# CornellHPC/HySortK

Measured on AMD Instinct MI355X. Metric: k-mers counted/sec at K=31, higher is better.
Workload: dtype u64

## Files before the change

hysortk_amd/csrc/hsk_device.h:

```cpp
#pragma once
#include <hip/hip_runtime.h>
#include <stdint.h>
#include "hsk_passplan.h"

namespace hsk {

typedef uint64_t u64;
typedef uint32_t u32;
typedef uint16_t u16;
typedef uint8_t u8;

constexpr int WAVE = 64;

__host__ __device__ __forceinline__ u64 rotl64(u64 x, int r) { return (x << r) | (x >> (64 - r)); }
__host__ __device__ __forceinline__ u64 fmix64(u64 k)
{
    k ^= k >> 33; k *= 0xff51afd7ed558ccdULL; k ^= k >> 33; k *= 0xc4ceb9fe1a85ec53ULL; k ^= k >> 33;
    return k;
}
__host__ __device__ __forceinline__ u64 murmur64_8(u64 key)
{
    u64 k1 = key * 0x87c37b91114253d5ULL;
    k1 = rotl64(k1, 31);
    k1 *= 0x4cf5ad432745937fULL;
    u64 h1 = 313ULL ^ k1, h2 = 313ULL;
    h1 ^= 8; h2 ^= 8;
    h1 += h2; h2 += h1;
    h1 = fmix64(h1); h2 = fmix64(h2);
    return h1 + h2;
}

template <int NW>
__host__ __device__ __forceinline__ u64 murmur64_words(const u64 (&w)[NW])
{
    if (NW == 1) return murmur64_8(w[0]);
    const u64 c1 = 0x87c37b91114253d5ULL, c2 = 0x4cf5ad432745937fULL;
    u64 h1 = 313ULL, h2 = 313ULL;
    u64 k1 = w[0], k2 = w[NW > 1 ? 1 : 0];
    k1 *= c1; k1 = rotl64(k1, 31); k1 *= c2; h1 ^= k1;
    h1 = rotl64(h1, 27); h1 += h2; h1 = h1 * 5 + 0x52dce729ULL;
    k2 *= c2; k2 = rotl64(k2, 33); k2 *= c1; h2 ^= k2;
    h2 = rotl64(h2, 31); h2 += h1; h2 = h2 * 5 + 0x38495ab5ULL;
    if (NW == 3) { u64 t1 = w[NW > 2 ? 2 : 0]; t1 *= c1; t1 = rotl64(t1, 31); t1 *= c2; h1 ^= t1; }
    h1 ^= (u64)(8 * NW); h2 ^= (u64)(8 * NW);
    h1 += h2; h2 += h1;
    h1 = fmix64(h1); h2 = fmix64(h2);
    return h1 + h2;
}

__host__ __device__ __forceinline__ u64 rev2(u64 x)
{
#if defined(__HIP_DEVICE_COMPILE__)
    x = __brevll(x);
#else
    x = ((x >> 1) & 0x5555555555555555ULL) | ((x & 0x5555555555555555ULL) << 1);
    x = ((x >> 2) & 0x3333333333333333ULL) | ((x & 0x3333333333333333ULL) << 2);
    x = ((x >> 4) & 0x0f0f0f0f0f0f0f0fULL) | ((x & 0x0f0f0f0f0f0f0f0fULL) << 4);
    x = __builtin_bswap64(x);
#endif
    return ((x >> 1) & 0x5555555555555555ULL) | ((x & 0x5555555555555555ULL) << 1);
}

__host__ __device__ __forceinline__ u64 twin1(u64 fw, int len)
{
    u64 t = ~rev2(fw);
    return t << (64 - 2 * len);
}

template <int NW> struct Mer { u64 w[NW]; };

template <int NW>
__host__ __device__ __forceinline__ Mer<NW> twin(const Mer<NW> &m, int k)
{
    Mer<NW> t;
#pragma unroll
    for (int l = 0; l < NW; ++l) t.w[NW - 1 - l] = ~rev2(m.w[l]);
    const int sh = (NW * 64 - 2 * k);
    if (sh) {
#pragma unroll
        for (int i = 0; i < NW; ++i) {
            u64 nxt = (i + 1 < NW) ? t.w[i + 1] : 0;
            t.w[i] = (t.w[i] << sh) | (nxt >> (64 - sh));
        }
    }
    return t;
}

template <int NW>
__host__ __device__ __forceinline__ bool mer_less(const Mer<NW> &a, const Mer<NW> &b)
{
#pragma unroll
    for (int i = 0; i < NW; ++i) {
        if (a.w[i] < b.w[i]) return true;
        if (a.w[i] > b.w[i]) return false;
    }
    return false;
}

template <int NW>
__host__ __device__ __forceinline__ Mer<NW> canonical(const Mer<NW> &m, int k)
{
    Mer<NW> t = twin<NW>(m, k);
    return mer_less<NW>(t, m) ? t : m;
}

__device__ __forceinline__ u64 bits64_be32(const u32 *words, u32 bit)
{
    u32 i = bit >> 5, s = bit & 31;
    u64 hi = ((u64)words[i] << 32) | words[i + 1];
    u64 lo = (u64)words[i + 2] << 32;
    return s ? ((hi << s) | (lo >> (64 - s))) : hi;
}

__device__ __forceinline__ u64 bits64_bytes(const u64 *p8, u64 bit)
{
    u64 i = bit >> 6; u32 s = (u32)(bit & 63);
    u64 hi = __builtin_bswap64(p8[i]);
    if (!s) return hi;
    u64 lo = __builtin_bswap64(p8[i + 1]);
    return (hi << s) | (lo >> (64 - s));
}
__device__ __forceinline__ u64 bits64_bytes_clamped(const u64 *p8, u64 bit, u64 nwords)
{
    u64 i = bit >> 6; u32 s = (u32)(bit & 63);
    u64 hi = i < nwords ? __builtin_bswap64(p8[i]) : 0;
    if (!s) return hi;
    u64 lo = (i + 1 < nwords) ? __builtin_bswap64(p8[i + 1]) : 0;
    return (hi << s) | (lo >> (64 - s));
}

struct FastMod { u32 d; u32 c16, c32, c48; u32 inv; };
inline FastMod make_fastmod(u32 d)
{
    FastMod f; f.d = d;
    f.c16 = d > 1 ? (u32)((1ULL << 16) % d) : 0; f.c32 = d > 1 ? (u32)((1ULL << 32) % d) : 0; f.c48 = d > 1 ? (u32)((1ULL << 48) % d) : 0;
    f.inv = d > 1 ? (u32)((1ULL << 32) / d) : 0;
    return f;
}
__host__ __device__ __forceinline__ u32 fastmod64(u64 x, const FastMod &f)
{
    if (f.d <= 1) return 0;
    const u32 a = (u32)(x >> 48), b = (u32)(x >> 32) & 0xFFFFu, c = (u32)(x >> 16) & 0xFFFFu, e = (u32)x & 0xFFFFu;
    const u32 t = a * f.c48 + b * f.c32 + c * f.c16 + e;
#if defined(__HIP_DEVICE_COMPILE__)
    const u32 q = __umulhi(t, f.inv);
#else
    const u32 q = (u32)(((u64)t * f.inv) >> 32);
#endif
    u32 r = t - q * f.d;
    if (r >= f.d) r -= f.d;
    if (r >= f.d) r -= f.d;
    return r;
}

__device__ __forceinline__ int lane_id() { return (int)__builtin_amdgcn_mbcnt_hi(~0u, __builtin_amdgcn_mbcnt_lo(~0u, 0)); }

__device__ __forceinline__ u32 wave_incl_scan_dpp(u32 v)
{
    v += (u32)__builtin_amdgcn_update_dpp(0, (int)v, 0x111, 0xF, 0xF, false);
    v += (u32)__builtin_amdgcn_update_dpp(0, (int)v, 0x112, 0xF, 0xF, false);
    v += (u32)__builtin_amdgcn_update_dpp(0, (int)v, 0x114, 0xF, 0xF, false);
    v += (u32)__builtin_amdgcn_update_dpp(0, (int)v, 0x118, 0xF, 0xF, false);
    v += (u32)__builtin_amdgcn_update_dpp(0, (int)v, 0x142, 0xA, 0xF, false);
    v += (u32)__builtin_amdgcn_update_dpp(0, (int)v, 0x143, 0xC, 0xF, false);
    return v;
}

template <typename T>
__device__ __forceinline__ T wave_incl_scan(T v)
{
    if constexpr (sizeof(T) == 4 && (T)(-1) > (T)0) return (T)wave_incl_scan_dpp((u32)v);
    const int lane = lane_id();
#pragma unroll
    for (int o = 1; o < WAVE; o <<= 1) {
        T n = __shfl_up(v, o, WAVE);
        if (lane >= o) v += n;
    }
    return v;
}

template <typename T>
__device__ __forceinline__ T block_excl_scan_256(T v, T *scratch, T *total)
{
    const int lane = lane_id(), w = threadIdx.x >> 6;
    T inc = wave_incl_scan(v);
    if (lane == WAVE - 1) scratch[w] = inc;
    __syncthreads();
    T base = 0, tot = 0;
#pragma unroll
    for (int i = 0; i < 4; ++i) { T s = scratch[i]; if (i < w) base += s; tot += s; }
    __syncthreads();
    if (total) *total = tot;
    return base + inc - v;
}

__device__ __forceinline__ void lds_barrier() { asm volatile("s_waitcnt lgkmcnt(0)\n\ts_barrier" ::: "memory"); }

template <typename T>
__device__ __forceinline__ T block_excl_scan_256_lds(T v, T *scratch, T *total)
{
    const int lane = lane_id(), w = threadIdx.x >> 6;
    T inc = wave_incl_scan(v);
    if (lane == WAVE - 1) scratch[w] = inc;
    lds_barrier();
    T base = 0, tot = 0;
#pragma unroll
    for (int i = 0; i < 4; ++i) { T s = scratch[i]; if (i < w) base += s; tot += s; }
    lds_barrier();
    if (total) *total = tot;
    return base + inc - v;
}


template <int NW> __device__ __forceinline__ u64 pick_word(const u64 *k, int word)
{
    if (NW == 1) return k[0];
    if (NW == 2) return word == 0 ? k[0] : k[1];
    return word == 0 ? k[0] : (word == 1 ? k[1] : k[NW - 1]);
}

__host__ __device__ __forceinline__ u64 splitmix64(u64 x)
{
    x += 0x9e3779b97f4a7c15ULL;
    x = (x ^ (x >> 30)) * 0xbf58476d1ce4e5b9ULL;
    x = (x ^ (x >> 27)) * 0x94d049bb133111ebULL;
    return x ^ (x >> 31);
}

}
```

hysortk_amd/csrc/hsk_parse.h:

```cpp
#pragma once
#include "hsk_device.h"
#include "hsk_parseplan.h"

namespace hsk {

constexpr int PARSE_THREADS = 256;
constexpr int PARSE_PPT = 8;
static_assert(PARSE_TILE == PARSE_THREADS * PARSE_PPT, "a tile is one pass of the workgroup: 2048 positions = 512 bytes");
constexpr int SUPERMER_CUT = 128;
constexpr int MAX_K = 95;
constexpr int HSK_MAX_TASKS = 1024;
constexpr int PARSE_HMAX = PARSE_TILE + 96;
constexpr int PARSE_RWIN = 64;
static_assert(PARSE_RWIN + PARSE_WORDS <= PARSE_THREADS, "scan_kernel prefetches the next tile with one lane per read-index entry and per word");

struct BinTable { u32 *cursor; u32 *map; u32 vmax; u32 cap_chunks; u32 *ctl; u32 *chunk_bin; ulonglong2 *items; u32 *subs; u32 *err; };

struct ParseArgs {
    const u8 *packed;
    u64 packed_bytes;
    const u64 *roff;
    const u32 *rlen;
    u64 nreads;
    int k, m;
    u32 ntasks;
    FastMod fm;
    u64 ntiles;
    u32 tiles_per_block;
    u32 nslabs, slab;
    u64 slab_tiles;
    u32 place_one;
    int64_t rid_base;
    u64 *blk_cnt;
    const u64 *blk_base;
    u8 *sm_len;
    u64 *sm_gpos;
    int32_t *dump_dest;
    u16 *dest_cache;
    u32 *tile_rec;
    u32 *tile_nrec;
    u32 rec_cap;
    u32 place_group;
    u32 *overflow;
    u32 *tile_r0;
    u32 *tile_sub;
    u32 *sm_sub;
    u32 item_maxk;
    const struct BinTable *bins;
    unsigned short *sm_sub16;
    u32 vt_shift;
    u64 *sm_item;
    const u8 *task_skip;
    u8 *sm_bytes;
    u32 *sm_boff;
    const u64 *task_base3;
    u32 *packed_copy;
    u32 drop_mask;
    unsigned long long *dropped;
};

enum ParseMode { PARSE_COUNT = 0, PARSE_EMIT = 1, PARSE_DUMP = 2 };

__device__ __forceinline__ u64 find_read(const u64 *roff, u64 lo, u64 hi, u64 b)
{
    while (lo < hi) {
        u64 mid = lo + (hi - lo + 1) / 2;
        if (roff[mid] <= b) lo = mid; else hi = mid - 1;
    }
    return lo;
}

__device__ __forceinline__ void supermer_runs(const u16 *s_dest, u64 *s_bnd, u32 (&runs)[PARSE_PPT])
{
    const int tid = threadIdx.x, lane = tid & 63, wave = tid >> 6;
    bool start[PARSE_PPT];
#pragma unroll
    for (int j = 0; j < PARSE_PPT; ++j) {
        const u32 p = j * PARSE_THREADS + tid;
        const u16 d = s_dest[p];
        const u16 dp = p ? s_dest[p - 1] : (u16)0xFFFF;
        const bool bnd = (d == 0xFFFF) || ((p & (SUPERMER_CUT - 1)) == 0) || (d != dp);
        start[j] = bnd && d != 0xFFFF;
        const u64 m = __ballot(bnd);
        if (lane == 0) s_bnd[j * 4 + wave] = m;
    }
    __syncthreads();
#pragma unroll
    for (int j = 0; j < PARSE_PPT; ++j) {
        runs[j] = 0;
        if (!start[j]) continue;
        const u32 p = j * PARSE_THREADS + tid;
        const u32 lim = (p | (SUPERMER_CUT - 1)) + 1;
        const u32 w = p >> 6;
        u64 m = ((p & 63) == 63) ? 0ULL : (s_bnd[w] & (~0ULL << ((p & 63) + 1)));
        u32 nb = lim;
        if (m) nb = w * 64 + (u32)__builtin_ctzll(m);
        else if ((w & 1) == 0) { const u64 m2 = s_bnd[w + 1]; if (m2) nb = (w + 1) * 64 + (u32)__builtin_ctzll(m2); }
        runs[j] = nb - p;
    }
}

template <int MW>
__device__ __forceinline__ u64 wide_mmer_hash(const u32 *s_words, u32 p, int M)
{
    Mer<MW> fw;
#pragma unroll
    for (int x = 0; x < MW; ++x) fw.w[x] = bits64_be32(s_words, 2u * p + 64u * (u32)x);
    fw.w[MW - 1] &= ~0ULL << (64 * MW - 2 * M);
    const Mer<MW> c = canonical<MW>(fw, M);
    return murmur64_words<MW>(c.w);
}

__device__ __forceinline__ u32 homopolymer_positions(const u32 *s_words, int tid, int K, u32 drop_mask)
{
    const u64 d0 = bits64_be32(s_words, 16u * (u32)tid), d1 = bits64_be32(s_words, 16u * (u32)tid + 64u);
    u32 dm = 0;
#pragma unroll
    for (int i = 0; i < PARSE_PPT; ++i) {
        const u64 hi = i ? ((d0 << (2 * i)) | (d1 >> (64 - 2 * i))) : d0, lo = d1 << (2 * i);
        const u32 b = (u32)(hi >> 62);
        const u64 pat = ((b & 1u) ? 0x5555555555555555ULL : 0ULL) | ((b & 2u) ? 0xAAAAAAAAAAAAAAAAULL : 0ULL);
        const bool same = K <= 32 ? ((hi ^ pat) >> (64 - 2 * K)) == 0 : (hi == pat && ((lo ^ pat) >> (128 - 2 * K)) == 0);
        if (same && ((drop_mask >> ((b == 1u || b == 2u) ? 1 : 0)) & 1u)) dm |= 1u << i;
    }
    return dm;
}

template <int MODE, bool EXT, bool DROP = false>
__global__ __launch_bounds__(PARSE_THREADS, 4) void parse_kernel(ParseArgs a)
{
    __shared__ u32 s_words[PARSE_WORDS];
    __shared__ u64 s_hash[PARSE_HMAX];
    __shared__ __attribute__((aligned(16))) u16 s_dest[PARSE_TILE + 8];
    __shared__ u64 s_rng[4];
    __shared__ u64 s_roff[PARSE_RWIN];
    __shared__ u32 s_rlen[PARSE_RWIN];
    __shared__ u64 s_bnd[PARSE_TILE / 64];
    __shared__ u32 s_scan[12];
    extern __shared__ __attribute__((aligned(16))) u64 s_cur[];

    u32 ndrop = 0;
    const int tid = threadIdx.x;
    const int K = a.k, M = a.m, W = K - M + 1;
    const u64 total_pos = a.packed_bytes * 4;

    if (MODE == PARSE_COUNT) {
        for (u32 i = tid; i < 2 * a.ntasks; i += PARSE_THREADS) s_cur[i] = 0;
    } else if (MODE == PARSE_EMIT) {
        for (u32 t = tid; t < a.ntasks; t += PARSE_THREADS) s_cur[t] = a.blk_base[((u64)blockIdx.x * a.ntasks + t) * 2];
    }
    __syncthreads();

    const u64 tile0 = (u64)blockIdx.x * a.tiles_per_block;
    if (tid == 0) s_rng[1] = (tile0 < a.ntiles) ? find_read(a.roff, 0, a.nreads - 1, (tile0 * PARSE_TILE) >> 2) : 0;
    __syncthreads();
    const u64 RINF = ~0ULL >> 2;
    for (u32 ti = 0; ti < a.tiles_per_block; ++ti) {
        const u64 tile = tile0 + ti;
        if (tile >= a.ntiles) break;
        const u64 gbase = tile * PARSE_TILE;
        const bool cached_emit = (MODE == PARSE_EMIT) && a.dest_cache != nullptr;
        const u64 bbase = gbase >> 2;

        if (!cached_emit) {
            const u32 *src = reinterpret_cast<const u32 *>(a.packed + bbase);
            const u64 left = a.packed_bytes - bbase;
            for (int i = tid; i < PARSE_WORDS; i += PARSE_THREADS) {
                u32 wv = 0;
                if ((u64)i * 4 + 4 <= left) wv = __builtin_bswap32(src[i]);
                else if ((u64)i * 4 < left) {
                    for (u64 b = (u64)i * 4; b < left; ++b) wv |= (u32)a.packed[bbase + b] << (24 - 8 * (b & 3));
                }
                s_words[i] = wv;
            }
        }
        if (!cached_emit && tid < PARSE_RWIN) {
            const u64 rb = s_rng[1];
            u64 blast = bbase + PARSE_TILE / 4 - 1;
            if (blast >= a.packed_bytes) blast = a.packed_bytes - 1;
            const u64 idx = rb + tid;
            const u64 off = (idx <= a.nreads) ? a.roff[idx] : RINF;
            s_roff[tid] = off;
            s_rlen[tid] = (idx < a.nreads) ? a.rlen[idx] : 0;
            const u32 c0 = (u32)__popcll(__ballot(idx < a.nreads && off <= bbase));
            const u32 c1 = (u32)__popcll(__ballot(idx < a.nreads && off <= blast));
            if (tid == 0) {
                u64 r0 = rb + c0 - 1, r1 = rb + c1 - 1;
                const bool fast = c1 < PARSE_RWIN;
                if (!fast) {
                    r0 = find_read(a.roff, rb, a.nreads - 1, bbase);
                    r1 = find_read(a.roff, r0, a.nreads - 1, blast);
                }
                s_rng[0] = r0; s_rng[1] = r1; s_rng[2] = rb; s_rng[3] = fast ? 1 : 0;
            }
        }
        __syncthreads();

        const int p0 = tid * PARSE_PPT;
        const bool cached = cached_emit;
        const u64 mmask = ~0ULL << (64 - 2 * (M < 32 ? M : 31));
        if (!cached) {
            if (M < 32) {
                for (int p = tid; p < PARSE_TILE + W - 1; p += PARSE_THREADS) {
                    u64 fw = bits64_be32(s_words, 2u * (u32)p) & mmask;
                    u64 tw = twin1(fw, M);
                    s_hash[p] = murmur64_8(tw < fw ? tw : fw);
                }
            } else if (M < 64) {
                for (int p = tid; p < PARSE_TILE + W - 1; p += PARSE_THREADS) s_hash[p] = wide_mmer_hash<2>(s_words, (u32)p, M);
            } else {
                for (int p = tid; p < PARSE_TILE + W - 1; p += PARSE_THREADS) s_hash[p] = wide_mmer_hash<3>(s_words, (u32)p, M);
            }
        }
        __syncthreads();

        u64 mn[PARSE_PPT];
        if (cached) {
#pragma unroll
            for (int i = 0; i < PARSE_PPT; ++i) mn[i] = 0;
        } else if (W >= PARSE_PPT) {
            u64 c = ~0ULL;
            for (int j = PARSE_PPT - 1; j <= W - 1; ++j) { u64 v = s_hash[p0 + j]; c = v < c ? v : c; }
            u64 suf = ~0ULL;
            mn[PARSE_PPT - 1] = c;
#pragma unroll
            for (int i = PARSE_PPT - 2; i >= 0; --i) { u64 v = s_hash[p0 + i]; suf = v < suf ? v : suf; mn[i] = suf < c ? suf : c; }
            u64 run = ~0ULL;
#pragma unroll
            for (int i = 1; i < PARSE_PPT; ++i) { u64 v = s_hash[p0 + W + i - 1]; run = v < run ? v : run; mn[i] = run < mn[i] ? run : mn[i]; }
        } else {
#pragma unroll
            for (int i = 0; i < PARSE_PPT; ++i) {
                u64 c = ~0ULL;
                for (int j = 0; j < W; ++j) { u64 v = s_hash[p0 + i + j]; c = v < c ? v : c; }
                mn[i] = c;
            }
        }
        if (!cached) {
            const u64 g0 = gbase + p0;
            const u64 rlo = s_rng[0], rhi = s_rng[1], rb = s_rng[2];
            const bool fast = s_rng[3] != 0;
            u64 r, rstart, rend, nxt;
            if (fast) {
                u32 lo = (u32)(rlo - rb), hi = (u32)(rhi - rb);
                const u64 b0 = g0 >> 2;
                while (lo < hi) { u32 mid = (lo + hi + 1) >> 1; if (s_roff[mid] <= b0) lo = mid; else hi = mid - 1; }
                r = rb + lo; rstart = s_roff[lo] * 4; rend = rstart + s_rlen[lo];
                nxt = (r + 1 < a.nreads) ? s_roff[lo + 1] * 4 : ~0ULL;
            } else {
                r = find_read(a.roff, rlo, rhi, g0 >> 2);
                rstart = a.roff[r] * 4; rend = rstart + a.rlen[r];
                nxt = (r + 1 < a.nreads) ? a.roff[r + 1] * 4 : ~0ULL;
            }
            const int HUGE = 1 << 30;
            auto rel = [&](u64 x) -> int { return x >= gbase + (u64)HUGE ? HUGE : (x < gbase ? ((gbase - x) >= (u64)HUGE ? -HUGE : -(int)(gbase - x)) : (int)(x - gbase)); };
            int rend_r = rel(rend), nxt_r = rel(nxt);
            const int total_r = rel(total_pos);
            u32 dmk = 0;
            if constexpr (DROP) dmk = homopolymer_positions(s_words, tid, K, a.drop_mask);
#pragma unroll
            for (int i = 0; i < PARSE_PPT; ++i) {
                const int g = p0 + i;
                while (g >= nxt_r) {
                    ++r; rstart = nxt;
                    if (fast) { const u32 j = (u32)(r - rb); rend = rstart + s_rlen[j]; nxt = (r + 1 < a.nreads) ? s_roff[j + 1] * 4 : ~0ULL; }
                    else { rend = rstart + a.rlen[r]; nxt = (r + 1 < a.nreads) ? a.roff[r + 1] * 4 : ~0ULL; }
                    rend_r = rel(rend); nxt_r = rel(nxt);
                }
                bool valid = (g < total_r) && (g + K <= rend_r);
                if (DROP && valid && ((dmk >> i) & 1u)) { valid = false; if (MODE == PARSE_COUNT) ++ndrop; }
                const u32 d = fastmod64(mn[i], a.fm);
                s_dest[p0 + i] = valid ? (u16)d : (u16)0xFFFF;
            }
        }
        if (cached) {
            const uint4 v = *reinterpret_cast<const uint4 *>(a.dest_cache + gbase + p0);
            *reinterpret_cast<uint4 *>(&s_dest[p0]) = v;
        } else if (MODE == PARSE_COUNT && a.dest_cache != nullptr) {
            *reinterpret_cast<uint4 *>(a.dest_cache + gbase + p0) = *reinterpret_cast<const uint4 *>(&s_dest[p0]);
        }
        __syncthreads();

        if (MODE == PARSE_DUMP) {
#pragma unroll
            for (int i = 0; i < PARSE_PPT; ++i) {
                u64 g = gbase + p0 + i;
                if (g < total_pos) { u16 d = s_dest[p0 + i]; a.dump_dest[g] = d == 0xFFFF ? -1 : (int32_t)d; }
            }
        } else if (MODE == PARSE_COUNT) {
            u32 runs[PARSE_PPT];
            supermer_runs(s_dest, s_bnd, runs);
#pragma unroll
            for (int j = 0; j < PARSE_PPT; ++j) {
                if (!runs[j]) continue;
                const u32 d = s_dest[j * PARSE_THREADS + tid];
                const u32 nk = runs[j];
                const u32 nb = (nk + K - 1 + 3) >> 2;
                atomicAdd((unsigned long long *)&s_cur[2 * d + 0], (1ULL << 40) | (unsigned long long)nk);
                atomicAdd((unsigned long long *)&s_cur[2 * d + 1], (unsigned long long)nb);
            }
        } else {
            u32 *s_srt = reinterpret_cast<u32 *>(s_hash);
            u32 *s_tcnt = reinterpret_cast<u32 *>(s_cur + a.ntasks);
            u32 *s_tpre = s_tcnt + a.ntasks;
            for (u32 t = tid; t < a.ntasks; t += PARSE_THREADS) s_tcnt[t] = 0;
            __syncthreads();
            u32 rec[PARSE_PPT], rnk[PARSE_PPT];
            {
                u32 runs[PARSE_PPT];
                supermer_runs(s_dest, s_bnd, runs);
#pragma unroll
                for (int j = 0; j < PARSE_PPT; ++j) {
                    rec[j] = 0xFFFFFFFFu;
                    if (!runs[j]) continue;
                    const u32 p = j * PARSE_THREADS + tid;
                    const u32 d = s_dest[p];
                    rec[j] = p | ((runs[j] - 1) << 11) | (d << 18);
                    rnk[j] = atomicAdd(&s_tcnt[d], 1u);
                }
            }
            __syncthreads();
            {
                u32 c4[4], sum = 0;
#pragma unroll
                for (int j = 0; j < 4; ++j) { const u32 t = tid * 4 + j; c4[j] = t < a.ntasks ? s_tcnt[t] : 0; sum += c4[j]; }
                u32 tot;
                u32 e = block_excl_scan_256<u32>(sum, s_scan, &tot);
#pragma unroll
                for (int j = 0; j < 4; ++j) { const u32 t = tid * 4 + j; if (t < a.ntasks) s_tpre[t] = e; e += c4[j]; }
                if (tid == 0) s_scan[8] = tot;
            }
            __syncthreads();
#pragma unroll
            for (int i = 0; i < PARSE_PPT; ++i)
                if (rec[i] != 0xFFFFFFFFu) s_srt[s_tpre[rec[i] >> 18] + rnk[i]] = rec[i];
            __syncthreads();
            const u32 nrec = s_scan[8];
            for (u32 i = tid; i < nrec; i += PARSE_THREADS) {
                const u32 r = s_srt[i];
                const u32 d = r >> 18;
                if (a.task_skip && a.task_skip[d]) continue;
                const u64 slot = s_cur[d] + (i - s_tpre[d]);
                a.sm_len[slot] = (u8)(((r >> 11) & 127) + K);
                a.sm_gpos[slot] = gbase + (u64)(r & 2047);
            }
            __syncthreads();
            for (u32 t = tid; t < a.ntasks; t += PARSE_THREADS) s_cur[t] += s_tcnt[t];
        }
        __syncthreads();
    }

    if (MODE == PARSE_COUNT) {
        for (u32 t = tid; t < a.ntasks; t += PARSE_THREADS) {
            u64 *o = a.blk_cnt + ((u64)blockIdx.x * a.ntasks + t) * 3;
            const u64 pk = s_cur[2 * t];
            o[0] = pk >> 40; o[1] = s_cur[2 * t + 1]; o[2] = pk & ((1ULL << 40) - 1);
        }
        if (DROP && a.dropped) {
            u32 v = ndrop;
            for (int o = 32; o > 0; o >>= 1) v += __shfl_down(v, o, WAVE);
            if (lane_id() == 0 && v) atomicAdd(a.dropped, (unsigned long long)v);
        }
    }
}

__global__ __launch_bounds__(PARSE_THREADS) void emit_kernel(ParseArgs a)
{
    __shared__ __attribute__((aligned(16))) u16 s_dest[PARSE_TILE + 8];
    __shared__ u32 s_srt[PARSE_TILE];
    __shared__ u64 s_bnd[PARSE_TILE / 64];
    __shared__ u32 s_scan[12];
    extern __shared__ __attribute__((aligned(16))) u64 s_cur[];
    const int tid = threadIdx.x;
    const int K = a.k;
    u32 *s_tcnt = reinterpret_cast<u32 *>(s_cur + a.ntasks);
    u32 *s_tpre = s_tcnt + a.ntasks;
    for (u32 t = tid; t < a.ntasks; t += PARSE_THREADS) s_cur[t] = a.blk_base[((u64)blockIdx.x * a.ntasks + t) * 2];
    __syncthreads();
    const u64 tile0 = (u64)blockIdx.x * a.tiles_per_block;
    uint4 nextv = make_uint4(0, 0, 0, 0);
    if (tile0 < a.ntiles) nextv = *reinterpret_cast<const uint4 *>(a.dest_cache + tile0 * PARSE_TILE + tid * PARSE_PPT);
    for (u32 ti = 0; ti < a.tiles_per_block; ++ti) {
        const u64 tile = tile0 + ti;
        if (tile >= a.ntiles) break;
        const u64 gbase = tile * PARSE_TILE;
        *reinterpret_cast<uint4 *>(&s_dest[tid * PARSE_PPT]) = nextv;
        if (ti + 1 < a.tiles_per_block && tile + 1 < a.ntiles)
            nextv = *reinterpret_cast<const uint4 *>(a.dest_cache + (gbase + PARSE_TILE) + tid * PARSE_PPT);
        for (u32 t = tid; t < a.ntasks; t += PARSE_THREADS) s_tcnt[t] = 0;
        __syncthreads();
        u32 rec[PARSE_PPT], rnk[PARSE_PPT];
        {
            u32 runs[PARSE_PPT];
            supermer_runs(s_dest, s_bnd, runs);
#pragma unroll
            for (int j = 0; j < PARSE_PPT; ++j) {
                rec[j] = 0xFFFFFFFFu;
                if (!runs[j]) continue;
                const u32 p = j * PARSE_THREADS + tid;
                const u32 d = s_dest[p];
                rec[j] = p | ((runs[j] - 1) << 11) | (d << 18);
                rnk[j] = atomicAdd(&s_tcnt[d], 1u);
            }
        }
        __syncthreads();
        {
            u32 c4[4], sum = 0;
#pragma unroll
            for (int j = 0; j < 4; ++j) { const u32 t = tid * 4 + j; c4[j] = t < a.ntasks ? s_tcnt[t] : 0; sum += c4[j]; }
            u32 tot;
            u32 e = block_excl_scan_256<u32>(sum, s_scan, &tot);
#pragma unroll
            for (int j = 0; j < 4; ++j) { const u32 t = tid * 4 + j; if (t < a.ntasks) s_tpre[t] = e; e += c4[j]; }
            if (tid == 0) s_scan[8] = tot;
        }
        __syncthreads();
#pragma unroll
        for (int i = 0; i < PARSE_PPT; ++i)
            if (rec[i] != 0xFFFFFFFFu) s_srt[s_tpre[rec[i] >> 18] + rnk[i]] = rec[i];
        __syncthreads();
        const u32 nrec = s_scan[8];
        for (u32 i = tid; i < nrec; i += PARSE_THREADS) {
            const u32 r = s_srt[i];
            const u32 d = r >> 18;
            if (a.task_skip && a.task_skip[d]) continue;
            const u64 slot = s_cur[d] + (i - s_tpre[d]);
            a.sm_len[slot] = (u8)(((r >> 11) & 127) + K);
            a.sm_gpos[slot] = gbase + (u64)(r & 2047);
        }
        __syncthreads();
        for (u32 t = tid; t < a.ntasks; t += PARSE_THREADS) s_cur[t] += s_tcnt[t];
        __syncthreads();
    }
}

constexpr int SCAN_MAX_M = 25;
constexpr u32 BIN_CHUNK = 8192;
constexpr unsigned PARSE_XCC_GETREG = 20u | (0u << 6) | (3u << 11);
constexpr u32 BIN_SPIN_LIMIT = 1u << 12;
constexpr u32 BIN_CUR_STRIDE = 32;

__device__ __forceinline__ u32 bin_reserve(const BinTable &a, u32 bin)
{
    return __hip_atomic_fetch_add(&a.cursor[(u64)bin * BIN_CUR_STRIDE], 1u, __ATOMIC_RELAXED, __HIP_MEMORY_SCOPE_WORKGROUP);
}
__device__ __forceinline__ u64 bin_slot(const BinTable &a, u32 bin, u32 p, unsigned long long *mc , u32 vt)
{
    typedef __attribute__((address_space(1))) u32 G32;
    u32 *const err = a.err;
    const u32 v = p / BIN_CHUNK, off = p % BIN_CHUNK;
    if (v >= a.vmax) { atomicOr(err, 256u); return ~0ULL; }
    if (off == BIN_CHUNK / 2) {
        if (v + 1 >= a.vmax) atomicOr(err, 256u);
        else {
            u32 nx = __hip_atomic_fetch_add(&a.ctl[0], 1u, __ATOMIC_RELAXED, __HIP_MEMORY_SCOPE_AGENT) + 1u;
            if (nx > a.cap_chunks) { atomicOr(err, 128u); nx = 0xFFFFFFFFu; }
            else a.chunk_bin[nx - 1u] = bin | ((v + 1u) << 13);
            __hip_atomic_store((G32 *)(a.map + (u64)bin * a.vmax + v + 1u), nx, __ATOMIC_RELAXED, __HIP_MEMORY_SCOPE_WORKGROUP);
        }
    }
    u32 ph;
    const unsigned long long e = mc[2u * vt];
    if ((u32)(e >> 32) == v && (u32)e != 0u) ph = (u32)e;
    else {
        G32 *mp = (G32 *)(a.map + (u64)bin * a.vmax + v);
        u32 spins = 0;
        while ((ph = __hip_atomic_load(mp, __ATOMIC_RELAXED, __HIP_MEMORY_SCOPE_AGENT)) == 0u) {
            if (++spins > BIN_SPIN_LIMIT) { atomicOr(err, 2u); ph = 0xFFFFFFFFu; break; }
            __builtin_amdgcn_s_sleep(1);
        }
        mc[2u * vt] = ((unsigned long long)v << 32) | ph;
    }
    if (ph == 0xFFFFFFFFu) return ~0ULL;
    return (u64)(ph - 1u) * BIN_CHUNK + off;
}
__global__ void bins_init_kernel(BinTable t, u32 nbins)
{
    const u32 b = blockIdx.x * blockDim.x + threadIdx.x;
    if (b < nbins) { t.map[(u64)b * t.vmax] = b + 1u; t.chunk_bin[b] = b; }
    if (b == 0) t.ctl[0] = nbins;
}
__device__ __forceinline__ void bin_store(const BinTable &a, u64 slot, u64 w0, u64 w1, u32 nk, u32 sub)
{
    if (slot == ~0ULL) return;
    a.items[slot] = make_ulonglong2(w0, (w1 & ~0xFFULL) | (u64)nk);
    a.subs[slot] = sub;
}

constexpr int SCAN_HSTRIDE = PARSE_THREADS + 16;
__device__ __forceinline__ int scan_hidx(int p) { return (p & 7) * SCAN_HSTRIDE + (p >> 3); }

#ifdef HSK_DIAG
__device__ unsigned long long g_scan_diag[16];
#endif
template <int KT, int MT, bool BINS = false, bool DROP = false>
__global__ __launch_bounds__(PARSE_THREADS, 4) void scan_kernel(ParseArgs a)
{
    __shared__ u32 s_words2[BINS ? 2 : 1][PARSE_WORDS];
    __shared__ uint2 s_pend[BINS ? 2 * PARSE_THREADS : 1];
    __shared__ __attribute__((aligned(16))) u64 s_hash[8 * SCAN_HSTRIDE];
    __shared__ u64 s_last[PARSE_THREADS];
    __shared__ u64 s_bmin[PARSE_THREADS];
    __shared__ __attribute__((aligned(8))) u8 s_v8[PARSE_THREADS];
    __shared__ __attribute__((aligned(8))) u8 s_bnd8[PARSE_THREADS + 16];
    __shared__ u16 s_plist[PARSE_TILE];
    __shared__ u64 s_rng[4];
    __shared__ u64 s_roff[PARSE_RWIN];
    __shared__ u32 s_rlen[PARSE_RWIN];
    __shared__ u32 s_scan[12];
    extern __shared__ __attribute__((aligned(16))) u64 s_cur[];

    const int tid = threadIdx.x;
    const int K = KT ? KT : a.k, M = MT ? MT : a.m, W = K - M + 1;
    const u64 mmask = ~0ULL << (64 - 2 * M);
    for (u32 i = tid; i < 2 * a.ntasks; i += PARSE_THREADS) s_cur[i] = 0;
    unsigned long long *s_mc = reinterpret_cast<unsigned long long *>(s_cur) + 1;
    u32 pend_pos0 = 0, pend_pos1 = 0, pend_mask = 0;
    const u64 tile0 = (u64)a.slab * a.slab_tiles + (u64)blockIdx.x * a.tiles_per_block;
    const u64 tile_end = (a.nslabs > 1 && ((u64)a.slab + 1) * a.slab_tiles < a.ntiles) ? ((u64)a.slab + 1) * a.slab_tiles : a.ntiles;
    if (tid == 0) s_rng[1] = (tile0 < a.ntiles) ? find_read(a.roff, 0, a.nreads - 1, (tile0 * PARSE_TILE) >> 2) : 0;
    __syncthreads();
    const u64 RINF = ~0ULL >> 2;
    const int p0 = tid * PARSE_PPT;
    const u32 maxk = a.item_maxk ? a.item_maxk : 16u;
    const u32 xcc_nvt = BINS ? (__builtin_amdgcn_s_getreg(PARSE_XCC_GETREG) & 7u) * a.ntasks : 0u;
    u32 pf0 = 0, pf1 = 0, pf2 = 0; bool pf_have = false;
    u32 ndrop = 0;

#ifdef HSK_DIAG
    unsigned long long dacc[6] = {0, 0, 0, 0, 0, 0};
#endif
    auto complete_pending = [&](const u32 *wprev) {
        const BinTable &bt = *a.bins;
        if (pend_mask & 1u) {
            const uint2 m = s_pend[tid]; const u32 pp = m.x & 2047u, vt = m.x >> 16;
            bin_store(bt, bin_slot(bt, xcc_nvt + vt, pend_pos0, s_mc, vt), bits64_be32(wprev, 2u * pp), bits64_be32(wprev, 2u * pp + 64u), (m.x >> 11) & 31u, m.y);
        }
        if (pend_mask & 2u) {
            const uint2 m = s_pend[PARSE_THREADS + tid]; const u32 pp = m.x & 2047u, vt = m.x >> 16;
            bin_store(bt, bin_slot(bt, xcc_nvt + vt, pend_pos1, s_mc, vt), bits64_be32(wprev, 2u * pp), bits64_be32(wprev, 2u * pp + 64u), (m.x >> 11) & 31u, m.y);
        }
        pend_mask = 0;
    };
    u32 wsel = 0;
    for (u32 ti = 0; ti < a.tiles_per_block; ++ti) {
        const u64 tile = tile0 + ti;
        if (tile >= tile_end) break;
        const u64 gbase = tile * PARSE_TILE;
        const u64 bbase = gbase >> 2;
        u32 *const s_words = s_words2[BINS ? wsel : 0u];
        const u32 *const s_wprev = s_words2[BINS ? (wsel ^ 1u) : 0u];
        if (BINS) wsel ^= 1u;
#ifdef HSK_DIAG
        unsigned long long sd[6];
        if (tid == 0) { unsigned long long t_ = __builtin_amdgcn_s_memtime(); sd[0] = t_; }
#endif

        if (pf_have) { if (tid >= PARSE_RWIN && tid < PARSE_RWIN + PARSE_WORDS) s_words[tid - PARSE_RWIN] = __builtin_bswap32(pf0); }
        else {
            const u32 *src = reinterpret_cast<const u32 *>(a.packed + bbase);
            const u64 left = a.packed_bytes - bbase;
            for (int i = tid; i < PARSE_WORDS; i += PARSE_THREADS) {
                u32 wv = 0;
                if ((u64)i * 4 + 4 <= left) wv = __builtin_bswap32(src[i]);
                else if ((u64)i * 4 < left) {
                    for (u64 b = (u64)i * 4; b < left; ++b) wv |= (u32)a.packed[bbase + b] << (24 - 8 * (b & 3));
                }
                s_words[i] = wv;
            }
        }
        if (tid < PARSE_RWIN) {
            const u64 rb = s_rng[1];
            u64 blast = bbase + PARSE_TILE / 4 - 1;
            if (blast >= a.packed_bytes) blast = a.packed_bytes - 1;
            const u64 idx = rb + tid;
            const u64 off = pf_have ? ((u64)pf0 | ((u64)pf1 << 32)) : ((idx <= a.nreads) ? a.roff[idx] : RINF);
            s_roff[tid] = off;
            s_rlen[tid] = pf_have ? pf2 : ((idx < a.nreads) ? a.rlen[idx] : 0);
            const u32 c0 = (u32)__popcll(__ballot(idx < a.nreads && off <= bbase));
            const u32 c1 = (u32)__popcll(__ballot(idx < a.nreads && off <= blast));
            if (tid == 0) {
                u64 r0 = rb + c0 - 1, r1 = rb + c1 - 1;
                const bool fast = c1 < PARSE_RWIN;
                if (!fast) {
                    r0 = find_read(a.roff, rb, a.nreads - 1, bbase);
                    r1 = find_read(a.roff, r0, a.nreads - 1, blast);
                }
                s_rng[0] = r0; s_rng[1] = r1; s_rng[2] = rb; s_rng[3] = fast ? 1 : 0;
                if (a.tile_r0) a.tile_r0[tile] = (u32)r0;
            }
        }
        lds_barrier();
        if (a.packed_copy && tid < PARSE_TILE / 16 && bbase + 4u * (u64)tid < a.packed_bytes)
            a.packed_copy[(bbase >> 2) + tid] = __builtin_bswap32(s_words[tid]);
        {
            const u64 nb = bbase + PARSE_TILE / 4;
            pf_have = (ti + 1 < a.tiles_per_block) && (tile + 1 < tile_end) && (nb + (u64)PARSE_WORDS * 4 <= a.packed_bytes);
            if (pf_have) {
                if (tid < PARSE_RWIN) {
                    const u64 idx = s_rng[1] + tid;
                    const u64 o_ = (idx <= a.nreads) ? a.roff[idx] : RINF;
                    pf0 = (u32)o_; pf1 = (u32)(o_ >> 32);
                    pf2 = (idx < a.nreads) ? a.rlen[idx] : 0;
                } else if (tid < PARSE_RWIN + PARSE_WORDS) pf0 = reinterpret_cast<const u32 *>(a.packed + nb)[tid - PARSE_RWIN];
            }
        }
#ifdef HSK_DIAG
        if (tid == 0) { unsigned long long t_ = __builtin_amdgcn_s_memtime(); sd[1] = t_; }
#endif

        u64 h[PARSE_PPT];
        {
            const u64 w0 = bits64_be32(s_words, 16u * (u32)tid);
            const u64 rw = ~rev2(w0);
#pragma unroll
            for (int i = 0; i < PARSE_PPT; ++i) {
                const u64 fw = (w0 << (2 * i)) & mmask;
                const u64 rc = (rw << (2 * (32 - M - i))) & mmask;
                h[i] = murmur64_8(rc < fw ? rc : fw);
            }
#pragma unroll
            for (int i = 0; i < PARSE_PPT; ++i) s_hash[i * SCAN_HSTRIDE + tid] = h[i];
            if (W >= 2 * PARSE_PPT) {
                u64 bm = h[0];
#pragma unroll
                for (int i = 1; i < PARSE_PPT; ++i) bm = h[i] < bm ? h[i] : bm;
                s_bmin[tid] = bm;
            }
            for (int e = PARSE_THREADS - 1 - tid; e < W - 1; e += PARSE_THREADS) {
                const int p = PARSE_TILE + e;
                const u64 fw = bits64_be32(s_words, 2u * (u32)p) & mmask;
                const u64 tw = twin1(fw, M);
                s_hash[scan_hidx(p)] = murmur64_8(tw < fw ? tw : fw);
            }
        }
        lds_barrier();
#ifdef HSK_DIAG
        if (tid == 0) { unsigned long long t_ = __builtin_amdgcn_s_memtime(); sd[2] = t_; }
#endif

        u64 mn[PARSE_PPT];
        if (W >= PARSE_PPT) {
            u64 c = h[PARSE_PPT - 1];
            const int nfull = (W - PARSE_PPT) / PARSE_PPT;
            int j = PARSE_PPT;
            if (nfull > 0 && tid + nfull < PARSE_THREADS) {
                for (int b = 1; b <= nfull; ++b) { const u64 v = s_bmin[tid + b]; c = v < c ? v : c; }
                j = PARSE_PPT * (nfull + 1);
            }
#pragma unroll 8
            for (; j <= W - 1; ++j) { const u64 v = s_hash[scan_hidx(p0 + j)]; c = v < c ? v : c; }
            mn[PARSE_PPT - 1] = c;
            u64 suf = ~0ULL;
#pragma unroll
            for (int i = PARSE_PPT - 2; i >= 0; --i) { suf = h[i] < suf ? h[i] : suf; mn[i] = suf < c ? suf : c; }
            u64 run = ~0ULL;
#pragma unroll
            for (int i = 1; i < PARSE_PPT; ++i) { const u64 v = s_hash[scan_hidx(p0 + W + i - 1)]; run = v < run ? v : run; mn[i] = run < mn[i] ? run : mn[i]; }
        } else {
#pragma unroll
            for (int i = 0; i < PARSE_PPT; ++i) {
                u64 c = ~0ULL;
                for (int j = 0; j < W; ++j) { const u64 v = s_hash[scan_hidx(p0 + i + j)]; c = v < c ? v : c; }
                mn[i] = c;
            }
        }
        u32 vmask = 0;
        {
            const u64 g0 = gbase + p0;
            const u64 rlo = s_rng[0], rhi = s_rng[1], rb = s_rng[2];
            const bool fast = s_rng[3] != 0;
            u64 r, rstart, rend, nxt;
            if (fast) {
                u32 lo = (u32)(rlo - rb), hi = (u32)(rhi - rb);
                const u64 b0 = g0 >> 2;
                while (lo < hi) { const u32 mid = (lo + hi + 1) >> 1; if (s_roff[mid] <= b0) lo = mid; else hi = mid - 1; }
                r = rb + lo; rstart = s_roff[lo] * 4; rend = rstart + s_rlen[lo];
                nxt = (r + 1 < a.nreads) ? s_roff[lo + 1] * 4 : ~0ULL;
            } else {
                r = find_read(a.roff, rlo, rhi, g0 >> 2);
                rstart = a.roff[r] * 4; rend = rstart + a.rlen[r];
                nxt = (r + 1 < a.nreads) ? a.roff[r + 1] * 4 : ~0ULL;
            }
            if (nxt >= g0 + PARSE_PPT) {
                const long long cnt = (long long)rend - (long long)K - (long long)g0 + 1;
                vmask = cnt <= 0 ? 0u : (cnt >= PARSE_PPT ? 0xFFu : ((1u << (u32)cnt) - 1u));
            } else {
                static_assert(PARSE_PPT == 8, "two bytes of bases per lane");
                const long long cnt_lo = (long long)rend - (long long)K - (long long)g0 + 1;
                vmask = cnt_lo <= 0 ? 0u : (cnt_lo >= 4 ? 0xFu : ((1u << (u32)cnt_lo) - 1u));
                do {
                    ++r; rstart = nxt;
                    if (fast) { const u32 j = (u32)(r - rb); rend = rstart + s_rlen[j]; nxt = (r + 1 < a.nreads) ? s_roff[j + 1] * 4 : ~0ULL; }
                    else { rend = rstart + a.rlen[r]; nxt = (r + 1 < a.nreads) ? a.roff[r + 1] * 4 : ~0ULL; }
                } while (nxt <= g0 + 4);
                const long long cnt_hi = (long long)rend - (long long)K - (long long)(g0 + 4) + 1;
                vmask |= (cnt_hi <= 0 ? 0u : (cnt_hi >= 4 ? 0xFu : ((1u << (u32)cnt_hi) - 1u))) << 4;
            }
        }
        if constexpr (DROP) {
            const u32 dm = homopolymer_positions(s_words, tid, K, a.drop_mask);
            ndrop += (u32)__popc(vmask & dm);
            vmask &= ~dm;
        }
        s_last[tid] = mn[PARSE_PPT - 1];
        s_v8[tid] = (u8)vmask;
        lds_barrier();
#ifdef HSK_DIAG
        if (tid == 0) { unsigned long long t_ = __builtin_amdgcn_s_memtime(); sd[3] = t_; }
#endif

        u32 start8 = 0;
        {
            u64 pm = tid ? s_last[tid - 1] : 0;
            const u32 pv = tid ? (u32)(s_v8[tid - 1] >> 7) : 0u;
            u32 neq8 = 0;
#pragma unroll
            for (int i = 0; i < PARSE_PPT; ++i) { neq8 |= (mn[i] != pm ? 1u : 0u) << i; pm = mn[i]; }
            const u32 cut8 = ((tid & (SUPERMER_CUT / PARSE_PPT - 1)) == 0) ? 1u : 0u;
            const u32 prev8 = (vmask << 1) | pv;
            const u32 bnd8 = (~vmask | cut8 | ~prev8 | neq8) & 0xFFu;
            s_bnd8[tid] = (u8)bnd8;
            if (tid == 0) s_scan[10] = 0;
            start8 = vmask & bnd8;
        }
        u32 nrec;
        u32 off = block_excl_scan_256_lds<u32>((u32)__popc(start8), s_scan, &nrec);
#pragma unroll
        for (int i = 0; i < PARSE_PPT; ++i)
            if ((start8 >> i) & 1) { s_hash[off] = mn[i]; s_plist[off] = (u16)(p0 + i); ++off; }
        lds_barrier();
#ifdef HSK_DIAG
        if (tid == 0) { unsigned long long t_ = __builtin_amdgcn_s_memtime(); sd[4] = t_; }
#endif

        if (BINS) complete_pending(s_wprev);
        {
            const u64 *bw = reinterpret_cast<const u64 *>(s_bnd8);
            u32 *trec = a.tile_rec + tile * (u64)a.rec_cap;
            for (u32 r = tid; r < nrec; r += PARSE_THREADS) {
                const u32 p = s_plist[r];
                u32 d = fastmod64(s_hash[r], a.fm);
                const u32 sub = (u32)((s_hash[r] * 0x9E3779B97F4A7C15ULL) >> 32);
                if (a.vt_shift) d = (d << a.vt_shift) | (sub >> (32u - a.vt_shift));
                const u32 w = p >> 6;
                const u64 m = ((p & 63) == 63) ? 0ULL : (bw[w] & (~0ULL << ((p & 63) + 1)));
                u32 nb = (p | (SUPERMER_CUT - 1)) + 1;
                if (m) nb = w * 64 + (u32)__builtin_ctzll(m);
                else if ((w & 1) == 0) { const u64 m2 = bw[w + 1]; if (m2) nb = (w + 1) * 64 + (u32)__builtin_ctzll(m2); }
                u32 nk = nb - p;
                if constexpr (BINS) {
                    const BinTable &bt = *a.bins;
                    const u32 bin = xcc_nvt + d;
                    for (u32 pp = p, rest = nk, first = 1u; rest; first = 0u) {
                        const u32 piece = rest < maxk ? rest : maxk;
                        atomicAdd((unsigned long long *)&s_cur[2 * d + 0], (1ULL << 40) | (unsigned long long)piece);
                        const u32 pos = bin_reserve(bt, bin);
                        if (first && r < 2u * PARSE_THREADS) {
                            s_pend[r] = make_uint2(pp | (piece << 11) | (d << 16), sub);
                            if (r < (u32)PARSE_THREADS) { pend_pos0 = pos; pend_mask |= 1u; } else { pend_pos1 = pos; pend_mask |= 2u; }
                        } else bin_store(bt, bin_slot(bt, bin, pos, s_mc, d), bits64_be32(s_words, 2u * pp), bits64_be32(s_words, 2u * pp + 64u), piece, sub);
                        pp += piece; rest -= piece;
                    }
                    continue;
                }
                if (a.tile_sub && nk > maxk) {
                    for (u32 pp = p + maxk, rest = nk - maxk; rest; ) {
                        const u32 piece = rest < maxk ? rest : maxk;
                        const u32 rx = nrec + atomicAdd(&s_scan[10], 1u);
                        atomicAdd((unsigned long long *)&s_cur[2 * d + 0], (1ULL << 40) | (unsigned long long)piece);
                        atomicAdd((unsigned long long *)&s_cur[2 * d + 1], (unsigned long long)((piece + K - 1 + 3) >> 2));
                        if (rx < a.rec_cap) { trec[rx] = pp | ((piece - 1) << 11) | (d << 18); a.tile_sub[tile * (u64)a.rec_cap + rx] = sub; }
                        pp += piece; rest -= piece;
                    }
                    nk = maxk;
                }
                atomicAdd((unsigned long long *)&s_cur[2 * d + 0], (1ULL << 40) | (unsigned long long)nk);
                atomicAdd((unsigned long long *)&s_cur[2 * d + 1], (unsigned long long)((nk + K - 1 + 3) >> 2));
                if (r < a.rec_cap) { trec[r] = p | ((nk - 1) << 11) | (d << 18); if (a.tile_sub) a.tile_sub[tile * (u64)a.rec_cap + r] = sub; }
            }
        }
        lds_barrier();
        if (tid == 0 && !BINS) {
            const u32 nall = nrec + s_scan[10];
            a.tile_nrec[tile] = nall;
            if (nall > a.rec_cap) atomicOr(a.overflow, 1u);
        }
#ifdef HSK_DIAG
        if (tid == 0) { unsigned long long t_ = __builtin_amdgcn_s_memtime(); sd[5] = t_; }
#endif
#ifdef HSK_DIAG
        if (tid == 0) { for (int q = 0; q < 5; ++q) dacc[q] += sd[q + 1] - sd[q]; dacc[5] += 1; }
#endif
    }
#ifdef HSK_DIAG
    if (tid == 0) { for (int q = 0; q < 5; ++q) atomicAdd(&g_scan_diag[q], dacc[q]); atomicAdd(&g_scan_diag[8], dacc[5]); }
#endif
    if (BINS) complete_pending(s_words2[BINS ? (wsel ^ 1u) : 0u]);
    if constexpr (DROP) {
        u32 v = ndrop;
        for (int o = 32; o > 0; o >>= 1) v += __shfl_down(v, o, WAVE);
        if (lane_id() == 0 && v) atomicAdd(a.dropped, (unsigned long long)v);
    }
    for (u32 t = tid; t < a.ntasks; t += PARSE_THREADS) {
        u64 *o = a.blk_cnt + ((u64)blockIdx.x * a.ntasks + t) * 3;
        const u64 pk = s_cur[2 * t];
        const u64 bytes_t = BINS ? 0ULL : s_cur[2 * t + 1];
        if (a.slab == 0 || a.place_one) { o[0] = pk >> 40; o[1] = bytes_t; o[2] = pk & ((1ULL << 40) - 1); }
        else { o[0] += pk >> 40; o[1] += bytes_t; o[2] += pk & ((1ULL << 40) - 1); }
    }
}

__global__ __launch_bounds__(PARSE_THREADS) void place_kernel(ParseArgs a)
{
    if (a.place_one && a.overflow && *(const volatile u32 *)a.overflow) return;
    constexpr int RPT = PLACE_MAX_REC / PARSE_THREADS;
    __shared__ u32 s_scan[12];
    __shared__ u32 s_go[20];
    extern __shared__ __attribute__((aligned(16))) u64 s_cur[];
    const int tid = threadIdx.x;
    const int K = a.k;
    u32 *s_tcnt = reinterpret_cast<u32 *>(s_cur + a.ntasks);
    u32 *s_tpre = s_tcnt + a.ntasks;
    u32 *s_srt = s_tpre + a.ntasks;
    for (u32 t = tid; t < a.ntasks; t += PARSE_THREADS) s_cur[t] = a.blk_base[((u64)blockIdx.x * a.ntasks + t) * 2];
    const u32 G = a.place_group;
    const u32 nsl = a.nslabs > 1 ? a.nslabs : 1;
    for (u32 sl = a.place_one ? a.slab : 0; sl < (a.place_one ? a.slab + 1 : nsl); ++sl) {
    const u64 tile0 = (u64)sl * a.slab_tiles + (u64)blockIdx.x * a.tiles_per_block;
    const u64 tile_end = (nsl > 1 && ((u64)sl + 1) * a.slab_tiles < a.ntiles) ? ((u64)sl + 1) * a.slab_tiles : a.ntiles;
    for (u32 t0 = 0; t0 < a.tiles_per_block; t0 += G) {
        const u64 tfirst = tile0 + t0;
        if (tfirst >= tile_end) break;
        u32 ng = a.tiles_per_block - t0; if (ng > G) ng = G;
        if (tfirst + ng > tile_end) ng = (u32)(tile_end - tfirst);
        __syncthreads();
        if (tid == 0) {
            u32 run = 0;
            for (u32 j = 0; j < ng; ++j) { s_go[j] = run; u32 n = a.tile_nrec[tfirst + j]; run += n < a.rec_cap ? n : a.rec_cap; }
            for (u32 j = ng; j <= 16; ++j) s_go[j] = run;
        }
        for (u32 t = tid; t < a.ntasks; t += PARSE_THREADS) s_tcnt[t] = 0;
        __syncthreads();
        const u32 total = s_go[16];
        u32 rec[RPT], rnk[RPT];
#pragma unroll
        for (int x = 0; x < RPT; ++x) {
            const u32 i = x * PARSE_THREADS + tid;
            rec[x] = 0xFFFFFFFFu;
            if (i < total) {
                u32 j = 0;
                while (j + 1 < ng && s_go[j + 1] <= i) ++j;
                const u32 r = a.tile_rec[(tfirst + j) * (u64)a.rec_cap + (i - s_go[j])];
                rec[x] = r | (j << 28);
                rnk[x] = atomicAdd(&s_tcnt[(r >> 18) & 1023u], 1u);
            }
        }
        __syncthreads();
        {
            u32 c4[4], sum = 0;
#pragma unroll
            for (int j = 0; j < 4; ++j) { const u32 t = tid * 4 + j; c4[j] = t < a.ntasks ? s_tcnt[t] : 0; sum += c4[j]; }
            u32 e = block_excl_scan_256<u32>(sum, s_scan, nullptr);
#pragma unroll
            for (int j = 0; j < 4; ++j) { const u32 t = tid * 4 + j; if (t < a.ntasks) s_tpre[t] = e; e += c4[j]; }
        }
        __syncthreads();
#pragma unroll
        for (int x = 0; x < RPT; ++x)
            if (rec[x] != 0xFFFFFFFFu) s_srt[s_tpre[(rec[x] >> 18) & 1023u] + rnk[x]] = rec[x];
        __syncthreads();
        for (u32 i = tid; i < total; i += PARSE_THREADS) {
            const u32 r = s_srt[i];
            const u32 d = (r >> 18) & 1023u;
            if (a.task_skip && a.task_skip[d]) continue;
            const u64 slot = s_cur[d] + (i - s_tpre[d]);
            a.sm_len[slot] = (u8)(((r >> 11) & 127) + K);
            a.sm_gpos[slot] = (tfirst + (r >> 28)) * PARSE_TILE + (u64)(r & 2047);
        }
        __syncthreads();
        for (u32 t = tid; t < a.ntasks; t += PARSE_THREADS) s_cur[t] += s_tcnt[t];
    }
    }
}

struct PlaceItemStep { u32 sl, t0, ng; u64 tfirst; bool ok; };
__global__ __launch_bounds__(PLACE_ITEM_THREADS) void place_items_kernel(ParseArgs a)
{
    if (a.place_one && a.overflow && *(const volatile u32 *)a.overflow) return;
    constexpr int RPT = PLACE_ITEM_REC / PLACE_ITEM_THREADS;
    constexpr int T = PLACE_ITEM_THREADS;
    constexpr int WPT = (PLACE_ITEM_WORDS + T - 1) / T;
    constexpr int LPR = (RPT + 5) / 6;
    static_assert(PLACE_ITEM_TILES <= 32, "a record's tile of the step takes 5 bits");
    __shared__ u32 s_w[16];
    __shared__ u32 s_go[PLACE_ITEM_TILES + 4];
    extern __shared__ __attribute__((aligned(16))) u64 s_cur[];
    const int tid = threadIdx.x;
    const u32 nt = a.ntasks;
    u32 *s_tcnt = reinterpret_cast<u32 *>(s_cur + nt);
    u32 *s_tpre = s_tcnt + nt;
    u64 *s_srt = reinterpret_cast<u64 *>(s_tpre + nt + (nt & 1u));
    u32 *s_words = reinterpret_cast<u32 *>(s_srt + PLACE_ITEM_REC);
    for (u32 t = tid; t < nt; t += T) s_cur[t] = a.blk_base[((u64)blockIdx.x * nt + t) * 2];
    const u32 G = a.place_group < PLACE_ITEM_TILES ? a.place_group : PLACE_ITEM_TILES;
    const u32 *p32 = reinterpret_cast<const u32 *>(a.packed);
    const u32 nsl = a.nslabs > 1 ? a.nslabs : 1;
    const u32 sl_end = a.place_one ? a.slab + 1 : nsl;
    const int lane = lane_id(), wv = tid >> 6;
    auto step_at = [&](u32 sl, u32 t0) {
        PlaceItemStep s = {0, 0, 0, 0, false};
        for (; sl < sl_end; ++sl, t0 = 0) {
            if (t0 >= a.tiles_per_block) continue;
            const u64 tile_end = (nsl > 1 && ((u64)sl + 1) * a.slab_tiles < a.ntiles) ? ((u64)sl + 1) * a.slab_tiles : a.ntiles;
            const u64 tfirst = (u64)sl * a.slab_tiles + (u64)blockIdx.x * a.tiles_per_block + t0;
            if (tfirst >= tile_end) continue;
            u32 ng = a.tiles_per_block - t0; if (ng > G) ng = G;
            if (tfirst + ng > tile_end) ng = (u32)(tile_end - tfirst);
            s.sl = sl; s.t0 = t0; s.ng = ng; s.tfirst = tfirst; s.ok = true;
            break;
        }
        return s;
    };
    auto load_nrec = [&](const PlaceItemStep &s) {
        u32 n = 0;
        if (tid < WAVE && s.ok && (u32)tid < s.ng) { n = a.tile_nrec[s.tfirst + tid]; n = n < a.rec_cap ? n : a.rec_cap; }
        return n;
    };
    auto write_go = [&](const PlaceItemStep &s, u32 n) {
        if (tid < WAVE) {
            const u32 inc = wave_incl_scan(n);
            if ((u32)tid < s.ng) s_go[tid] = inc - n;
            const u32 tot = __shfl(inc, WAVE - 1);
            if ((u32)tid >= s.ng && (u32)tid <= PLACE_ITEM_TILES) s_go[tid] = tot;
        }
    };
    u32 rec[RPT], rnk[RPT], sub[RPT], lop[LPR], words[WPT];
    auto fetch = [&](const PlaceItemStep &s, u32 total) {
#pragma unroll
        for (int q = 0; q < LPR; ++q) lop[q] = 0;
#pragma unroll
        for (int x = 0; x < RPT; ++x) {
            const u32 i = x * T + tid;
            rec[x] = 0; sub[x] = 0;
            if (i < total) {
                u32 lo = 0, hi = s.ng;
                while (hi - lo > 1) { const u32 mid = (lo + hi) >> 1; if (s_go[mid] <= i) lo = mid; else hi = mid; }
                const u64 at = (s.tfirst + lo) * (u64)a.rec_cap + (i - s_go[lo]);
                rec[x] = a.tile_rec[at];
                sub[x] = a.tile_sub[at];
                lop[x / 6] |= lo << (5 * (x % 6));
            }
        }
        const u64 w0 = s.tfirst * (PARSE_TILE / 16);
        const u32 nw = s.ng * (PARSE_TILE / 16) + 8;
#pragma unroll
        for (int q = 0; q < WPT; ++q) {
            const u32 i = q * T + tid;
            words[q] = 0;
            if (i < nw) {
                const u64 b = (w0 + i) * 4;
// ... 438 lines not shown
```

Measured before the change: 90.33 billion.

## Use f64 min instructions for u64 minimizer scan and right-aligned hash keys

```diff
diff --git a/hysortk_amd/csrc/hsk_device.h b/hysortk_amd/csrc/hsk_device.h
--- a/hysortk_amd/csrc/hsk_device.h
+++ b/hysortk_amd/csrc/hsk_device.h
@@ -18,9 +18,10 @@
     k ^= k >> 33; k *= 0xff51afd7ed558ccdULL; k ^= k >> 33; k *= 0xc4ceb9fe1a85ec53ULL; k ^= k >> 33;
     return k;
 }
-__host__ __device__ __forceinline__ u64 murmur64_8(u64 key)
-{
-    u64 k1 = key * 0x87c37b91114253d5ULL;
+constexpr u64 MURMUR_C1 = 0x87c37b91114253d5ULL;
+__host__ __device__ __forceinline__ u64 murmur64_8_c1(u64 key, u64 c1s)
+{
+    u64 k1 = key * c1s;
     k1 = rotl64(k1, 31);
     k1 *= 0x4cf5ad432745937fULL;
     u64 h1 = 313ULL ^ k1, h2 = 313ULL;
@@ -29,6 +30,7 @@
     h1 = fmix64(h1); h2 = fmix64(h2);
     return h1 + h2;
 }
+__host__ __device__ __forceinline__ u64 murmur64_8(u64 key) { return murmur64_8_c1(key, MURMUR_C1); }
 
 template <int NW>
 __host__ __device__ __forceinline__ u64 murmur64_words(const u64 (&w)[NW])
diff --git a/hysortk_amd/csrc/hsk_fmin.h b/hysortk_amd/csrc/hsk_fmin.h
--- /dev/null
+++ b/hysortk_amd/csrc/hsk_fmin.h
@@ -0,0 +1,39 @@
+#pragma once
+#include <stdint.h>
+#include <string.h>
+
+#if defined(__HIPCC__)
+#define HSK_FMIN_HD __host__ __device__ __forceinline__
+#else
+#define HSK_FMIN_HD inline
+#endif
+
+namespace hsk {
+
+constexpr uint32_t FMIN_SENTINEL = 0x7FEFFFFFu;
+
+HSK_FMIN_HD uint64_t fmin_clamp(uint64_t v)
+{
+    const uint32_t hi = (uint32_t)(v >> 32);
+    return ((uint64_t)(hi < FMIN_SENTINEL ? hi : FMIN_SENTINEL) << 32) | (uint32_t)v;
+}
+
+HSK_FMIN_HD uint64_t fmin_u64(uint64_t a, uint64_t b)
+{
+#if defined(__HIP_DEVICE_COMPILE__)
+    double d;
+    asm("v_min_f64 %0, %1, %2" : "=v"(d) : "v"(__longlong_as_double((long long)a)), "v"(__longlong_as_double((long long)b)));
+    return (uint64_t)__double_as_longlong(d);
+#else
+    double x, y;
+    memcpy(&x, &a, 8); memcpy(&y, &b, 8);
+    const double m = y < x ? y : x;
+    uint64_t r;
+    memcpy(&r, &m, 8);
+    return r;
+#endif
+}
+
+HSK_FMIN_HD bool fmin_exact(uint64_t m) { return (uint32_t)(m >> 32) < FMIN_SENTINEL; }
+
+}
diff --git a/hysortk_amd/csrc/hsk_parse.h b/hysortk_amd/csrc/hsk_parse.h
--- a/hysortk_amd/csrc/hsk_parse.h
+++ b/hysortk_amd/csrc/hsk_parse.h
@@ -1,5 +1,6 @@
 #pragma once
 #include "hsk_device.h"
+#include "hsk_fmin.h"
 #include "hsk_parseplan.h"
 
 namespace hsk {
@@ -490,6 +491,39 @@
 constexpr int SCAN_HSTRIDE = PARSE_THREADS + 16;
 __device__ __forceinline__ int scan_hidx(int p) { return (p & 7) * SCAN_HSTRIDE + (p >> 3); }
 
+#ifndef HSK_SCAN_FMIN
+#define HSK_SCAN_FMIN 1
+#endif
+#ifndef HSK_SCAN_RKEY
+#define HSK_SCAN_RKEY 1
+#endif
+
+template <bool FAST>
+__device__ __forceinline__ void scan_window_minima(const u64 (&h)[PARSE_PPT], const u64 *s_hash, const u64 *s_bmin, int tid, int W, u64 (&mn)[PARSE_PPT])
+{
+    auto in = [](u64 v) -> u64 { return FAST ? fmin_clamp(v) : v; };
+    auto lower = [](u64 x, u64 y) -> u64 { return FAST ? fmin_u64(x, y) : (y < x ? y : x); };
+    const int p0 = tid * PARSE_PPT;
+    u64 c = in(h[PARSE_PPT - 1]);
+    const int nfull = (W - PARSE_PPT) / PARSE_PPT;
+    int j = PARSE_PPT;
+    if (nfull > 0 && tid + nfull < PARSE_THREADS) {
+        for (int b = 1; b <= nfull; ++b) c = lower(c, in(s_bmin[tid + b]));
+        j = PARSE_PPT * (nfull + 1);
+    }
+#pragma unroll 8
+    for (; j <= W - 1; ++j) c = lower(c, in(s_hash[scan_hidx(p0 + j)]));
+    mn[PARSE_PPT - 1] = c;
+    u64 suf = in(h[PARSE_PPT - 2]);
+    mn[PARSE_PPT - 2] = lower(suf, c);
+#pragma unroll
+    for (int i = PARSE_PPT - 3; i >= 0; --i) { suf = lower(suf, in(h[i])); mn[i] = lower(suf, c); }
+    u64 run = in(s_hash[scan_hidx(p0 + W)]);
+    mn[1] = lower(run, mn[1]);
+#pragma unroll
+    for (int i = 2; i < PARSE_PPT; ++i) { run = lower(run, in(s_hash[scan_hidx(p0 + W + i - 1)])); mn[i] = lower(run, mn[i]); }
+}
+
 #ifdef HSK_DIAG
 __device__ unsigned long long g_scan_diag[16];
 #endif
@@ -512,6 +546,7 @@
 
     const int tid = threadIdx.x;
     const int K = KT ? KT : a.k, M = MT ? MT : a.m, W = K - M + 1;
+    constexpr bool FIXED_KM = KT != 0 && MT != 0;
     const u64 mmask = ~0ULL << (64 - 2 * M);
     for (u32 i = tid; i < 2 * a.ntasks; i += PARSE_THREADS) s_cur[i] = 0;
     unsigned long long *s_mc = reinterpret_cast<unsigned long long *>(s_cur) + 1;
@@ -613,11 +648,21 @@
         {
             const u64 w0 = bits64_be32(s_words, 16u * (u32)tid);
             const u64 rw = ~rev2(w0);
-#pragma unroll
-            for (int i = 0; i < PARSE_PPT; ++i) {
-                const u64 fw = (w0 << (2 * i)) & mmask;
-                const u64 rc = (rw << (2 * (32 - M - i))) & mmask;
-                h[i] = murmur64_8(rc < fw ? rc : fw);
+            if constexpr (HSK_SCAN_RKEY && FIXED_KM) {
+                const u64 kmask = ~0ULL >> (64 - 2 * M), c1s = MURMUR_C1 << (64 - 2 * M);
+#pragma unroll
+                for (int i = 0; i < PARSE_PPT; ++i) {
+                    const u64 fw = (w0 >> (64 - 2 * M - 2 * i)) & kmask;
+                    const u64 rc = (rw >> (2 * i)) & kmask;
+                    h[i] = murmur64_8_c1(fmin_u64(rc, fw), c1s);
+                }
+            } else {
+#pragma unroll
+                for (int i = 0; i < PARSE_PPT; ++i) {
+                    const u64 fw = (w0 << (2 * i)) & mmask;
+                    const u64 rc = (rw << (2 * (32 - M - i))) & mmask;
+                    h[i] = murmur64_8(rc < fw ? rc : fw);
+                }
             }
 #pragma unroll
             for (int i = 0; i < PARSE_PPT; ++i) s_hash[i * SCAN_HSTRIDE + tid] = h[i];
@@ -641,22 +686,13 @@
 
         u64 mn[PARSE_PPT];
         if (W >= PARSE_PPT) {
-            u64 c = h[PARSE_PPT - 1];
-            const int nfull = (W - PARSE_PPT) / PARSE_PPT;
-            int j = PARSE_PPT;
-            if (nfull > 0 && tid + nfull < PARSE_THREADS) {
-                for (int b = 1; b <= nfull; ++b) { const u64 v = s_bmin[tid + b]; c = v < c ? v : c; }
-                j = PARSE_PPT * (nfull + 1);
-            }
-#pragma unroll 8
-            for (; j <= W - 1; ++j) { const u64 v = s_hash[scan_hidx(p0 + j)]; c = v < c ? v : c; }
-            mn[PARSE_PPT - 1] = c;
-            u64 suf = ~0ULL;
-#pragma unroll
-            for (int i = PARSE_PPT - 2; i >= 0; --i) { suf = h[i] < suf ? h[i] : suf; mn[i] = suf < c ? suf : c; }
-            u64 run = ~0ULL;
-#pragma unroll
-            for (int i = 1; i < PARSE_PPT; ++i) { const u64 v = s_hash[scan_hidx(p0 + W + i - 1)]; run = v < run ? v : run; mn[i] = run < mn[i] ? run : mn[i]; }
+            if constexpr (HSK_SCAN_FMIN && FIXED_KM) {
+                scan_window_minima<true>(h, s_hash, s_bmin, tid, W, mn);
+                u32 top = (u32)(mn[0] >> 32);
+#pragma unroll
+                for (int i = 1; i < PARSE_PPT; ++i) { const u32 t = (u32)(mn[i] >> 32); top = t > top ? t : top; }
+                if (__ballot(top >= FMIN_SENTINEL)) scan_window_minima<false>(h, s_hash, s_bmin, tid, W, mn);
+            } else scan_window_minima<false>(h, s_hash, s_bmin, tid, W, mn);
         } else {
 #pragma unroll
             for (int i = 0; i < PARSE_PPT; ++i) {
```

After: 92.20 billion, median of 6. 1.02x the previous value.
